# LeSN-Lab/diff-ViT

Measured on AMD Instinct MI355X. Metric: images/sec DeiT-S int8 224^2 b=256 (quantized forward), higher is better.
Workload: dtype int8; 1 GPU; deit_small PoT-PTQ forward, bit_config=[8]*50, 224x224, batch 256 per GPU; global_batch=256, parallelism=dp1, streams_per_gpu=3, collective=none, ranks_seen=1, distinct_devices=1

## Files before the change

diff-vit_amd/csrc/p2vit_attn.hip:

```cpp
#include "p2vit_attn_lis.h"

#define WA_HD 32
#define WA_KEYS 64
#define WA_DEAD(kb, r) (NT > 0 && (kb) * 16 + (r) >= NT)
#define WA_PAD(kb, r) (!(NT > 0 && (kb) * 16 + 12 + (r) < NT))
template <int NT, bool TAP>
__global__ __launch_bounds__(256, 3) void k_window_attention(WinAttnArgs a) {
  constexpr int VSTRIDE = WA_KEYS + 4;
  __shared__ __attribute__((aligned(16))) int8_t sK[4][WA_KEYS * WA_HD];
  __shared__ __attribute__((aligned(16))) unsigned short sVt[4][WA_HD * VSTRIDE];
  __shared__ float sT[4][232];
  __shared__ __attribute__((aligned(16))) unsigned short sP[4][4][16];
  __shared__ unsigned short sMeta[WA_KEYS + 16];
  __shared__ long long lutE[258];
  __shared__ double lutFR[258];
  const int tid = threadIdx.x, lane = tid & 63, wave = tid >> 6, g = lane >> 4, l15 = lane & 15;
  const int ws = a.wa.ws, N = ws * ws, nW = a.wa.n_windows;
  const int hgroups = (a.H + 3) >> 2;
  const int blk = blockIdx.x;
  const int hg = blk % hgroups, w = (blk / hgroups) % nW, b = blk / (hgroups * nW);
  const int head = hg * 4 + wave;
  const int C = a.H * WA_HD;
  const long long ldq = a.wa.qkv_stride ? a.wa.qkv_stride : 3 * C, ldo = a.wa.out_stride ? a.wa.out_stride : C;
  const bool hok = head < a.H;
// ... 244 lines not shown
  const int hgroups = (a.H + 3) / 4;
  const dim3 grid((unsigned)(a.B * a.wa.n_windows * hgroups));
  if (a.wa.ws == 7) {
    if (a.probs_k) hipLaunchKernelGGL((k_window_attention<49, true>), grid, dim3(256), 0, st, a);
    else hipLaunchKernelGGL((k_window_attention<49, false>), grid, dim3(256), 0, st, a);
  } else {
    if (a.probs_k) hipLaunchKernelGGL((k_window_attention<0, true>), grid, dim3(256), 0, st, a);
    else hipLaunchKernelGGL((k_window_attention<0, false>), grid, dim3(256), 0, st, a);
  }
  CHECK_LAUNCH();
  return 0;
}

int p2v_launch_attention_wide(const AttnArgs& a, int head_dim, int nkb, hipStream_t st);

int g_attn_stream = 0;
int p2v_launch_attention(const AttnArgs& a, int head_dim, hipStream_t st) {
  const int nkb = (a.N + 31) / 32;
  {
    int ex;
    const float m2 = a.at.s_qkv_sq * a.at.inv_s_attn;
    if (!(m2 > 0.f) || frexpf(m2, &ex) != 0.5f) return -2;
  }
  if (g_attn_stream || a.N > p2v_resident_tokens_of(head_dim)) return p2v_launch_attention_stream(a, head_dim, st);
  if (head_dim == 64) { P2V_ATTN_CASES(64, 19, true) }
  if (head_dim == 32) { P2V_ATTN_CASES(32, 19, false) }
  return p2v_launch_attention_wide(a, head_dim, nkb, st);
}
```

diff-vit_amd/csrc/p2vit_attn_lis.h:

```cpp
#pragma once
#include "p2vit_device.h"

extern int g_attn_waves;


#define P2V_PROB_SCALE 0x1p111f
__device__ __forceinline__ unsigned lis_prob_pair(float r0, float r1) {
  const unsigned hi2 = __builtin_amdgcn_perm(__float_as_uint(r1), __float_as_uint(r0), 0x07060302u);
  const unsigned eb = __builtin_bit_cast(unsigned, __builtin_bit_cast(v2u16, hi2) + (v2u16){0x40, 0x40}) & 0x7F807F80u;
  unsigned out;
  asm("v_pk_sub_u16 %0, %1, %2 clamp" : "=v"(out) : "s"(0x47804780u), "v"(eb));
  return out;
}

#ifdef P2V_DIAG
extern unsigned long long* g_gemm_stamps;
#define AT_STAMP(slot)                                                                                             \
  do {                                                                                                             \
    if (a.stamps && threadIdx.x == 0 && (slot) < 16) a.stamps[(long long)blockIdx.x * 16 + (slot)] = __builtin_readcyclecounter(); \
  } while (0)
#else
#define AT_STAMP(slot) do { } while (0)
#endif
template <int HD, int NKP, bool TAP, bool ISH>
__global__ __launch_bounds__(512, HD > 64 ? 2 : (NKP <= 7 ? 4 : (NKP <= 10 ? 3 : 2))) void k_lis_attention(AttnArgs a) {
  static_assert(HD % 16 == 0 && HD >= 16 && HD <= 128, "head_dim");
  constexpr int KROWS = NKP * 32;
  constexpr int NKB = NKP * 2;
  constexpr int VSTRIDE = KROWS + 4;
// ... 3 lines not shown
  extern __shared__ __attribute__((aligned(16))) unsigned char smem[];
  int8_t* sK = reinterpret_cast<int8_t*>(smem);
  unsigned short* sVt = reinterpret_cast<unsigned short*>(smem + KROWS * HD);
  unsigned char* lutE = smem + KROWS * HD + HD * VSTRIDE * 2;
  unsigned char* lutFR = lutE + 258 * 8;
  typedef __attribute__((address_space(3))) const long long* lds_i64p;
  typedef __attribute__((address_space(3))) const double* lds_f64p;
  const int ebase = (int)(unsigned)(uintptr_t)(__attribute__((address_space(3))) unsigned char*)lutE;

  const int tid = threadIdx.x, lane = tid & 63, wave = tid >> 6, g = lane >> 4, l15 = lane & 15;
  const int b = blockIdx.x / a.H, head = blockIdx.x % a.H;
  const int N = a.N, D = a.H * HD, ld = 3 * D;
  const int8_t* base = a.qkv + (long long)b * N * ld + head * HD;
  AT_STAMP(0);

  if (tid < 256) {
    int xi = -tid;
    const int lim = 32 * a.at.x0_int;
    xi = xi < lim ? lim : xi;
    const int q = xi / a.at.x0_int;
    const int r = xi - a.at.x0_int * q;
    const long long z = (long long)r * (r + a.at.b_int) + a.at.c_int;
    long long e = z << (32 - q);
    e = e < 0 ? 0 : e;
    const float ef = (float)e;
    reinterpret_cast<long long*>(lutE)[tid] = e;
    reinterpret_cast<double*>(lutFR)[tid] = 1.0 / (double)ef;
    if (tid == 0) {
      reinterpret_cast<long long*>(lutE)[256] = 0;
      reinterpret_cast<double*>(lutFR)[256] = 1.0;
    }
  }
  AT_STAMP(1);
  for (int i0 = tid; i0 < KROWS * CH; i0 += 2 * (int)blockDim.x) {
    uint4 kv[2], vv[2];
#pragma unroll
    for (int u = 0; u < 2; ++u) {
      const int i = i0 + u * (int)blockDim.x;
      const int row = i / CH, c = i % CH;
      kv[u] = make_uint4(0, 0, 0, 0);
      vv[u] = make_uint4(0, 0, 0, 0);
      if (i < KROWS * CH && row < N) {
        kv[u] = *reinterpret_cast<const uint4*>(base + (long long)row * ld + D + c * 16);
        vv[u] = *reinterpret_cast<const uint4*>(base + (long long)row * ld + 2 * D + c * 16);
      }
    }
#pragma unroll
    for (int u = 0; u < 2; ++u) {
      const int i = i0 + u * (int)blockDim.x;
      if (i >= KROWS * CH) break;
      const int row = i / CH, c = i % CH;
      const int sw = (HD == 64) ? (c ^ (((row >> 3) & 1) << 1)) : c;
      *reinterpret_cast<uint4*>(sK + row * HD + sw * 16) = kv[u];
      const unsigned w4[4] = {vv[u].x, vv[u].y, vv[u].z, vv[u].w};
#pragma unroll
      for (int j = 0; j < 16; ++j) {
        const float f = (float)sx8(w4[j >> 2], j & 3);
        sVt[(c * 16 + j) * VSTRIDE + row] = (unsigned short)(__float_as_uint(f) >> 16);
      }
// ... 31 lines not shown
    v4i s[NKB];
#pragma unroll
    for (int kb = 0; kb < NKB; ++kb) {
      const int row = kb * 16 + l15;
#pragma unroll
      for (int j = 0; j < NQ; ++j) {
        const bool live = 4 * j + g < CH;
        const int c = live ? 4 * j + g : 0;
        const int sw = (HD == 64) ? (c ^ (((row >> 3) & 1) << 1)) : c;
        v4i fk = *reinterpret_cast<const v4i*>(sK + row * HD + sw * 16);
        if (!live) fk = (v4i){0, 0, 0, 0};
        if (j == 0) s[kb] = __builtin_amdgcn_mfma_i32_16x16x64_i8(fk, fq[0], (v4i){0, 0, 0, 0}, 0, 0, 0);
        else s[kb] = __builtin_amdgcn_mfma_i32_16x16x64_i8(fk, fq[j], s[kb], 0, 0, 0);
      }
    }
    const bool tail_empty = (NKB - 1) * 16 >= N;
#ifdef P2V_DIAG
    asm volatile("s_nop 0" :: "v"(s[NKB - 1][0]));
#endif
    AT_STAMP(stamp_base);
    long long S = 0;
    if (ISH) {
      const int p = a.pshift, hm1 = (1 << (p - 1)) - 1;
      int mx = -100000;
#pragma unroll
      for (int kb = 0; kb < NKB; ++kb) {
        if (kb == NKB - 1 && tail_empty) continue;
#pragma unroll
        for (int r = 0; r < 4; ++r) {
          const int sv = s[kb][r];
          int code = (int)((unsigned)sv + (unsigned)hm1 + (((unsigned)sv >> p) & 1u)) >> p;
          code = code < -128 ? -128 : (code > 127 ? 127 : code);
          if (kb >= NKB - 2) code = (kb * 16 + 4 * g + r) < N ? code : -100000;
          s[kb][r] = code;
          mx = code > mx ? code : mx;
        }
      }
      {
        int o = __shfl_xor(mx, 16);
        mx = o > mx ? o : mx;
        o = __shfl_xor(mx, 32);
        mx = o > mx ? o : mx;
      }
      const int mx8 = (mx << 3) + ebase;
#pragma unroll
      for (int kb = 0; kb < NKB; ++kb) {
        if (kb == NKB - 1 && tail_empty) continue;
#pragma unroll
        for (int r = 0; r < 4; ++r) {
          int d8;
          asm("v_mad_i32_i24 %0, %1, -8, %2" : "=v"(d8) : "v"(s[kb][r]), "v"(mx8));
          if (kb >= NKB - 2) d8 = d8 > ebase + 2048 ? ebase + 2048 : d8;
          s[kb][r] = d8;
          S += *(lds_i64p)(uintptr_t)(unsigned)d8;
        }
        __builtin_amdgcn_sched_barrier(0);
      }
    } else {
    int mn = 1000;
#pragma unroll
    for (int kb = 0; kb < NKB; ++kb) {
      if (kb == NKB - 1 && tail_empty) continue;
#pragma unroll
      for (int r = 0; r < 4; ++r) {
        int nc = (int)__builtin_amdgcn_fmed3f(rintf((float)s[kb][r] * nmm), -127.f, 128.f);
        if (kb >= NKB - 2) nc = (kb * 16 + 4 * g + r) < N ? nc : 1000;
        s[kb][r] = nc;
        mn = nc < mn ? nc : mn;
      }
    }
    {
      int o = __shfl_xor(mn, 16);
      mn = o < mn ? o : mn;
      o = __shfl_xor(mn, 32);
      mn = o < mn ? o : mn;
    }
    const int neg8mn = -8 * mn + ebase;
#pragma unroll
    for (int kb = 0; kb < NKB; ++kb) {
      if (kb == NKB - 1 && tail_empty) continue;
#pragma unroll
      for (int r = 0; r < 4; ++r) {
        int d8 = (s[kb][r] << 3) + neg8mn;
        if (kb >= NKB - 2) d8 = d8 > ebase + 2048 ? ebase + 2048 : d8;
        s[kb][r] = d8;
        S += *(lds_i64p)(uintptr_t)(unsigned)d8;
      }
      __builtin_amdgcn_sched_barrier(0);
    }
    }
    S += __shfl_xor(S, 16);
    S += __shfl_xor(S, 32);
    const float Sf = (float)S;
    const double Sd = (double)Sf;
    AT_STAMP(stamp_base + 1);

    v4f o[NDT];
#pragma unroll
    for (int dt = 0; dt < NDT; ++dt) o[dt] = (v4f){0.f, 0.f, 0.f, 0.f};
#pragma unroll
    for (int p = 0; p < NKP; ++p) {
      unsigned pk[4];
#pragma unroll
      for (int e2 = 0; e2 < 4; ++e2) {
        float ratio[2];
#pragma unroll
        for (int e = 0; e < 2; ++e) {
          const int j = 2 * e2 + e;
          const int kb = 2 * p + (j >> 2), r = j & 3;
          if (kb == NKB - 1 && tail_empty) {
            ratio[e] = 4.0e9f;
            continue;
          }
          const double rd = ((lds_f64p)(uintptr_t)(unsigned)s[kb][r])[258];
          ratio[e] = rintf((float)(Sd * rd));
          if (TAP && s[kb][r] < ebase + 2048 && qrow < N) {
            int k = (int)((__float_as_uint(ratio[e]) + 0x00400000u) >> 23) - 127;
            a.probs_k[(((long long)b * a.H + head) * N + qrow) * N + kb * 16 + 4 * g + r] = (int8_t)(k > 16 ? 16 : k);
          }
        }
        pk[e2] = lis_prob_pair(ratio[0], ratio[1]);
      }
      v4i pb = {(int)pk[0], (int)pk[1], (int)pk[2], (int)pk[3]};
      const v8bf fb = __builtin_bit_cast(v8bf, pb);
#pragma unroll
      for (int dt = 0; dt < NDT; ++dt) {
        const unsigned short* vp = sVt + (dt * 16 + l15) * VSTRIDE + p * 32 + 4 * g;
        const uint2 lo = *reinterpret_cast<const uint2*>(vp);
        const uint2 hi = *reinterpret_cast<const uint2*>(vp + 16);
        v4i va = {(int)lo.x, (int)lo.y, (int)hi.x, (int)hi.y};
        o[dt] = __builtin_amdgcn_mfma_f32_16x16x32_bf16(__builtin_bit_cast(v8bf, va), fb, o[dt], 0, 0, 0);
      }
      __builtin_amdgcn_sched_barrier(0);
    }
#ifdef P2V_DIAG
    asm volatile("s_nop 0" :: "v"(o[NDT - 1][0]));
#endif
    AT_STAMP(stamp_base + 2);
    {
      const int qs = qrow < N ? qrow : N - 1;
      int8_t* dst = a.out + ((long long)b * N + qs) * D + head * HD + 4 * g;
#pragma unroll
      for (int dt = 0; dt < NDT; ++dt)
        *reinterpret_cast<unsigned*>(dst + dt * 16) = pack4_rne_sat(o[dt][0] * avm, o[dt][1] * avm, o[dt][2] * avm, o[dt][3] * avm);
    }
    AT_STAMP(stamp_base + 3);
    stamp_base += 4;
  }
}

template <int HD, int NKB, bool ISH_OK = true>
static int launch_attn_t(const AttnArgs& a_, hipStream_t st) {
  constexpr int KROWS = NKB * 32;
  constexpr size_t smem = (size_t)KROWS * HD + (size_t)HD * (KROWS + 4) * 2 + 258 * 8 + 258 * 8;
  AttnArgs a = a_;
  {
    int ex;
    const float m = a.at.qk_scale * (a.at.s_qkv_sq * a.at.inv_s_attn);
    a.pshift = (m > 0.f && frexpf(m, &ex) == 0.5f && ex <= 0 && ex >= -23) ? 1 - ex : 0;
  }
#ifdef P2V_DIAG
  a.stamps = g_gemm_stamps;
#endif
// ... 40 lines not shown
```

diff-vit_amd/csrc/p2vit_capi.cpp:

```cpp
#include <hip/hip_runtime.h>
#include <math.h>
#include <stdarg.h>
#include <stdio.h>
#include <stdlib.h>
#include <string.h>

#include <vector>

#include "p2vit_kernels.h"

static thread_local char g_err[512] = "";

static int fail(int code, const char* fmt, ...) {
  va_list ap;
  va_start(ap, fmt);
  vsnprintf(g_err, sizeof g_err, fmt, ap);
  va_end(ap);
  return code;
}
static int launch_rc(int rc, const char* what) {
  if (rc == 0) return 0;
  if (rc == -2) return fail(P2V_E_UNSUPPORTED, "%s: s_qkv_sq * inv_s_attn must be a power of two", what);
  if (rc < 0) return fail(P2V_E_UNSUPPORTED, "%s: no kernel instantiated for this shape", what);
  return fail(P2V_E_LAUNCH, "%s: %s", what, hipGetErrorString((hipError_t)rc));
// ... 37 lines not shown
  std::vector<char> lin_set[2];
  float inv_s_input;
  p2v_epilogue embed_epi;
  const int8_t* cls_codes;
  bool embed_set;
  std::vector<p2v_block> blocks;
  std::vector<char> block_set;
  p2v_ln final_ln;
  float head_inv_s, head_s;
  bool head_set;
  std::vector<float*> ln_pre_buf;
  float* final_pre_buf = nullptr;
  std::vector<char> block_folded;
  std::vector<const float*> resid_tab;
  std::vector<float*> resid_buf;
  int device = -1;
  ~p2v_plan() {
    int prev = -1;
    const bool sw = device >= 0 && hipGetDevice(&prev) == hipSuccess && prev != device && hipSetDevice(device) == hipSuccess;
    for (float* b : ln_pre_buf)
      if (b) (void)hipFree(b);
    for (float* b : resid_buf)
      if (b) (void)hipFree(b);
    if (final_pre_buf) (void)hipFree(final_pre_buf);
    if (sw) (void)hipSetDevice(prev);
  }
};

static void build_resid_tables(p2v_plan* plan, int block);
static int bit_index(int bits) { return bits == 4 ? 0 : (bits == 8 ? 1 : -1); }

extern "C" {

extern int g_ln_generic;
extern int g_ln_rows;
extern int g_attn_waves;
extern int g_ln_gemm;
extern int g_ln_gemm_ver;
extern int g_gemm_tile;
extern int g_resid_pre;
extern int g_attn_stream;
extern int g_ln_pre;
extern int g_gemm_rows;
int g_cls_rows = 1;
// ... 70 lines not shown
  p->patches = (d.img_size / d.patch_size) * (d.img_size / d.patch_size);
  p->tokens = p->patches + 1;
  p->k_patch = d.in_chans * d.patch_size * d.patch_size;
  p->k_patch_pad = round_up(p->k_patch, GBK_PAD);
  p->n_layers = 4 * d.depth + 2;
  for (int b = 0; b < 2; ++b) {
    p->lin[b].assign(p->n_layers, p2v_linear{nullptr, nullptr, nullptr, nullptr, 0});
    p->lin_set[b].assign(p->n_layers, 0);
  }
  p->blocks.resize(d.depth);
  p->block_set.assign(d.depth, 0);
  p->ln_pre_buf.assign(d.depth, nullptr);
  p->block_folded.assign(d.depth, 0);
  p->resid_tab.assign((size_t)d.depth * 4, nullptr);
  p->resid_buf.assign(d.depth, nullptr);
  p->embed_set = p->head_set = false;
  p->cls_codes = nullptr;
  *out = p;
  return P2V_OK;
}

void p2v_plan_destroy(p2v_plan* plan) { delete plan; }

int p2v_plan_set_linear(p2v_plan* plan, int layer, int bits, const p2v_linear* lin) {
  if (!plan || !lin) return fail(P2V_E_ARG, "p2v_plan_set_linear: null argument");
  const int bi = bit_index(bits);
  if (bi < 0) return fail(P2V_E_BITS, "bits %d not in {4, 8}", bits);
  if (layer < 0 || layer >= plan->n_layers) return fail(P2V_E_ARG, "layer %d out of range [0,%d)", layer, plan->n_layers);
  if (!lin->w_codes || !lin->colscale || !lin->bias) return fail(P2V_E_ARG, "p2v_plan_set_linear: null device pointer");
  if (lin->packed4 && bits != 4) return fail(P2V_E_BITS, "packed4 weights for a %d-bit layer", bits);
// ... 70 lines not shown
  const size_t per = resid_tab_floats(D);
  if (hipDeviceSynchronize() != hipSuccess) { (void)hipGetLastError(); return; }
  float* buf = plan->resid_buf[block];
  if (!buf && hipMalloc(&buf, 4 * per * sizeof(float)) != hipSuccess) { (void)hipGetLastError(); return; }
  plan->resid_buf[block] = buf;
  plan->device = dev.own;
  for (int which = 0; which < 2; ++which)
    for (int bi = 0; bi < 2; ++bi) {
      const int layer = 1 + 4 * block + (which ? 3 : 1);
      if (!plan->lin_set[bi][layer]) continue;
      int usable = 0;
      float* tab = buf + (size_t)(which * 2 + bi) * per;
      if (resid_prefold_impl(plan->lin[bi][layer], which ? blk.fc2_epi : blk.proj_epi, D, tab, &usable, nullptr) == P2V_OK && usable)
        plan->resid_tab[(size_t)block * 4 + which * 2 + bi] = tab;
    }
}

static hipError_t fold_one_ln(const p2v_ln& l, int C, float* dev, p2v_ln_pre* out) {
  const int Cp = round_up(C, 256);
  std::vector<float> g(C), b(C), io(C), pm(C), host((size_t)2 * Cp, 0.f);
  hipError_t e = hipMemcpy(g.data(), l.gamma, C * sizeof(float), hipMemcpyDeviceToHost);
  if (e == hipSuccess) e = hipMemcpy(b.data(), l.beta, C * sizeof(float), hipMemcpyDeviceToHost);
  if (e == hipSuccess) e = hipMemcpy(io.data(), l.inv_out, C * sizeof(float), hipMemcpyDeviceToHost);
  if (e == hipSuccess) e = hipMemcpy(pm.data(), l.post_mul, C * sizeof(float), hipMemcpyDeviceToHost);
  if (e != hipSuccess) return e;
  float* go = host.data();
  float* bo = go + Cp;
  int pot = 1, pm1 = 1;
  float gmin = 3.0e38f, gmax = 0.f, bmax = 0.f;
  for (int c = 0; c < C; ++c) {
// ... 61 lines not shown
                       !blk->fc2_epi.s_next))
    rc = fail(P2V_E_ARG, "p2v_plan_set_block: RESID epilogues need s_mid/s_res/s_next");
  for (int i = 0; i < 6 && rc == P2V_OK; ++i) {
    const p2v_ln& l = i < 2 ? blk->ln1[i] : blk->ln2[(i - 2) >> 1][(i - 2) & 1];
    if (!l.mask || !l.gamma || !l.beta || !l.inv_out || !l.post_mul) rc = fail(P2V_E_ARG, "p2v_plan_set_block: LayerNorm constants missing");
  }
  if (rc != P2V_OK) return rc;
  plan->blocks[block] = *blk;
  plan->block_set[block] = 1;
  g_err[0] = 0;
  plan->block_folded[block] = fold_ln_constants(plan, block) ? 1 : 0;
  {
    char keep[sizeof g_err];
    memcpy(keep, g_err, sizeof keep);
    build_resid_tables(plan, block);
    memcpy(g_err, keep, sizeof keep);
  }
  return P2V_OK;
}

int p2v_plan_block_prefolded(const p2v_plan* plan, int block) {
  if (!plan || block < 0 || block >= plan->d.depth) return fail(P2V_E_ARG, "p2v_plan_block_prefolded: bad argument");
  return plan->block_folded[block] ? 1 : 0;
}

int p2v_plan_resid_prefolded(const p2v_plan* plan, int block) {
  if (!plan || block < 0 || block >= plan->d.depth) return fail(P2V_E_ARG, "p2v_plan_resid_prefolded: bad argument");
  int m = 0;
  for (int j = 0; j < 4; ++j) m |= plan->resid_tab[(size_t)block * 4 + j] ? 1 << j : 0;
  return m;
}

int p2v_plan_set_head(p2v_plan* plan, const p2v_ln* final_ln, float inv_s_out, float s_out) {
// ... 228 lines not shown
    LnArgs ln{bufX, D, M, D, b.ln1[bq], bufLN, D};
    ln.pre = b.ln1[bq].pre;
    p2v_epilogue e{};
    e.inv_s_out = b.inv_s_qkv[bq];
    e.tap_out = qkv_tap ? qkv_tap[i] : (lin_tap ? lin_tap[1 + 4 * i] : nullptr);
    if (p->lin[bq][1 + 4 * i].w_frag && p2v_ln_gemm_supported(P2V_EPI_REQUANT, D, 3 * D, 0)) {
      if (!taps) ln.out = nullptr;
      STEP(P2V_K_LN_GEMM_QKV, run_ln_gemm(P2V_EPI_REQUANT, ln, p->lin[bq][1 + 4 * i], e, 3 * D, bufQKV, st));
    } else {
      STEP(P2V_K_LAYERNORM, launch_rc(p2v_launch_layernorm(ln, st), "int_layernorm"));
      STEP(P2V_K_GEMM_QKV, run_gemm(P2V_EPI_REQUANT, bufLN, D, M, Dk, 3 * D, p->lin[bq][1 + 4 * i], e, bufQKV, 3 * D, nullptr, st));
    }
    DDV_TAP(T, 3 * D);
    DDV_I8(bufQKV, T, 3 * D, nullptr);
    AttnArgs at{bufQKV, batch, T, d.num_heads, b.attn, bufATT, nullptr};
    p2v_epilogue ep = b.proj_epi;
    ep.residual = bufX;
    ep.resid_tab = p->resid_tab[(size_t)i * 4 + bp];
    if (i == d.depth - 1 && cls_only) {
      const long long TD = (long long)T * D;
      at.nq = 1;
      STEP(P2V_K_ATTENTION, launch_rc(p2v_launch_attention(at, hd, st), "lis_attention"));
      STEP(P2V_K_GEMM_PROJ, run_gemm_few_rows(P2V_EPI_RESID, bufATT, (int)TD, batch, Dk, D, p->lin[bp][2 + 4 * i], ep, bufX, (int)TD, st));
      LnArgs lc{bufX, TD, batch, D, b.ln2[bq][b1], bufLN, D};
      lc.pre = b.ln2[bq][b1].pre;
      STEP(P2V_K_LAYERNORM, launch_rc(p2v_launch_layernorm(lc, st), "int_layernorm"));
      p2v_epilogue e1{};
      e1.inv_s_out = b.inv_s_fc1;
      e1.gelu = b.gelu_fc1;
      STEP(P2V_K_GEMM_FC1, run_gemm_few_rows(P2V_EPI_GELU, bufLN, D, batch, Dk, Hd, p->lin[b1][3 + 4 * i], e1, bufHID, Hd, st));
// ... 252 lines not shown

int p2v_lis_attention_rows(const int8_t* qkv, int batch, int tokens, int heads, int head_dim, const p2v_attn* at, int query_rows,
                           int8_t* out, void* stream) {
  if (!qkv || !at || !out) return fail(P2V_E_ARG, "p2v_lis_attention_rows: null argument");
  if (batch <= 0 || tokens <= 0 || heads <= 0) return fail(P2V_E_SHAPE, "bad attention shape");
  if (query_rows < 1 || query_rows > tokens) return fail(P2V_E_SHAPE, "p2v_lis_attention_rows: query_rows %d outside 1 .. %d", query_rows, tokens);
  {
    const int rc = check_attn("p2v_lis_attention_rows", *at);
    if (rc != P2V_OK) return rc;
  }
  AttnArgs a{qkv, batch, tokens, heads, *at, out, nullptr};
  a.nq = query_rows;
  return launch_rc(p2v_launch_attention(a, head_dim, (hipStream_t)stream), "lis_attention");
}

int p2v_patch_merge_gather(const int8_t* x, int batch, int H, int W, int C, int8_t* out, void* stream) {
  if (!x || !out) return fail(P2V_E_ARG, "p2v_patch_merge_gather: null argument");
  if (batch <= 0 || H <= 0 || W <= 0 || (H & 1) || (W & 1)) return fail(P2V_E_SHAPE, "patch merge: H and W must be positive and even");
  if (C <= 0 || C % 16) return fail(P2V_E_UNSUPPORTED, "patch merge: C must be a multiple of 16");
  return launch_rc(p2v_launch_patch_merge_gather(x, batch, H, W, C, out, (hipStream_t)stream), "patch_merge_gather");
}

int p2v_avgpool_quant(const int8_t* x, int batch, int tokens, int C, float s_in, float inv_s_out, int8_t* out, void* stream) {
  if (!x || !out) return fail(P2V_E_ARG, "p2v_avgpool_quant: null argument");
  if (batch <= 0 || tokens <= 0 || tokens > 8192) return fail(P2V_E_SHAPE, "avgpool: bad shape");
  if (C <= 0 || C % 4) return fail(P2V_E_UNSUPPORTED, "avgpool: C must be a multiple of 4");
  return launch_rc(p2v_launch_avgpool_quant(x, batch, tokens, C, s_in, inv_s_out, out, (hipStream_t)stream), "avgpool_quant");
}

int p2v_window_attention(const int8_t* qkv, int batch, int tokens_per_image, int heads, int head_dim, const p2v_winattn* wa,
// ... 269 lines not shown
```

diff-vit_amd/csrc/p2vit_kernels.h:

```cpp
#pragma once
#include <hip/hip_runtime.h>
#include <stdint.h>

#include "../../include/p2vit.h"

#define GBK_PAD 64
#define P2V_EPI_F32 7

struct GemmArgs {
  const int8_t* A;
  int lda, M;
  const int8_t* W;
  int K, N;
  int w4;
  const float* colscale;
  const float* bias;
  p2v_epilogue ep;
  void* out;
  int ldo;
  int8_t* out_codes;
  int tiles_n;
#ifdef P2V_DIAG
  unsigned long long* stamps;
#endif
// ... 10 lines not shown
  int8_t* out;
  long long out_stride;
  int rows_per_half;
  int force_generic;
  LnPre pre;
};

struct AttnArgs {
  const int8_t* qkv;
  int B, N, H;
  p2v_attn at;
  int8_t* out;
  int8_t* probs_k;
  int pshift;
  int nq;
#ifdef P2V_DIAG
  unsigned long long* stamps;
#endif
};

struct WinAttnArgs {
  const int8_t* qkv;
  int B, T, H;
  p2v_winattn wa;
  int8_t* out;
  int8_t* probs_k;
};
int p2v_launch_patch_merge_gather(const int8_t* x, int B, int H, int W, int C, int8_t* out, hipStream_t st);
int p2v_launch_avgpool_quant(const int8_t* x, int B, int T, int C, float s_in, float inv_s_out, int8_t* out, hipStream_t st);
int p2v_launch_window_attention(const WinAttnArgs& a, hipStream_t st);

int p2v_launch_patchify(const float* img, int B, int C, int H, int W, int P, float inv_s, int8_t* out, int k_pad, hipStream_t st);
int p2v_launch_fill_cls(int8_t* x, int B, int T, int D, const int8_t* cls, hipStream_t st);
int p2v_launch_embed_fp32(const float* img, int B, int C, int H, int W, int P, const GemmArgs& g, hipStream_t st);
int p2v_launch_u8_patchify(const uint8_t* img, int B, int C, int H, int W, int P, int nhwc, const int8_t* lut, int8_t* out, int k_pad,
                           hipStream_t st);
int p2v_launch_embed_u8(const uint8_t* img, int nhwc, const float* lut, int B, int C, int H, int W, int P, const GemmArgs& g, hipStream_t st);
int p2v_launch_gemm(int epi, const GemmArgs& g, hipStream_t st);
int p2v_launch_gemm_rows(int epi, const GemmArgs& g, hipStream_t st);
int p2v_launch_resid_prefold(const p2v_linear& lin, const p2v_epilogue& ep, int N, float* tab, unsigned* flags, hipStream_t st);
int p2v_launch_layernorm(const LnArgs& a, hipStream_t st);
bool p2v_ln_gemm_supported(int epi, int C, int N, int table_cells);
int p2v_launch_ln_gemm(int epi, const LnArgs& a, const GemmArgs& g, hipStream_t st);
int p2v_launch_attention(const AttnArgs& a, int head_dim, hipStream_t st);
int p2v_launch_attention_stream(const AttnArgs& a, int head_dim, hipStream_t st);
inline int p2v_resident_tokens_of(int head_dim) {
  if (head_dim == 32 || head_dim == 48 || head_dim == 64 || head_dim == 80) return P2V_MAX_TOKENS;
  return head_dim == 96 ? 17 * 32 : (head_dim == 128 ? 12 * 32 : 0);
}
int p2v_launch_stream_probe(int kernels, int usec, int workgroups, int lds_bytes, hipStream_t st);
int p2v_launch_fake_quant(const float* x, long long n, const float* scale, int n_scale, long long inner, int lo, int hi,
                          float* out, int8_t* codes, hipStream_t st);
int p2v_launch_gelu_quant(const float* y, long long n, float inv_s, int8_t* codes, unsigned long long* flags, int force_slow,
                          hipStream_t st);
int p2v_launch_gelu_sweep(unsigned first_bits, unsigned count, float* max_err, hipStream_t st);
int p2v_launch_gelu_table_build(float inv_s, const p2v_gelu_tab& t, unsigned* scratch, hipStream_t st);
int p2v_launch_gelu_table_check(float inv_s, const p2v_gelu_tab& t, unsigned long long* mismatches, hipStream_t st);

#include <vector>
// ... 37 lines not shown
```

diff-vit_amd/engine.py:

```python
import ctypes as C
import os

_HERE = os.path.dirname(os.path.abspath(__file__))
LIB_PATH = os.path.join(_HERE, 'csrc', 'libp2vit_hip.so')

P2V_ABI_VERSION = 6
EPI_REQUANT, EPI_GELU, EPI_RESID, EPI_EMBED, EPI_HEAD = 0, 1, 2, 3, 4
E_ARG, E_BITS, E_SHAPE, E_UNSUPPORTED, E_WORKSPACE, E_LAUNCH, E_STATE = -1, -2, -3, -4, -5, -6, -7
LAYOUT_NCHW, LAYOUT_NHWC = 0, 1
LAYOUTS = {'NCHW': LAYOUT_NCHW, 'NHWC': LAYOUT_NHWC}

KERNEL_KINDS = ('patchify', 'gemm_embed', 'fill_cls', 'layernorm', 'gemm_qkv', 'attention', 'gemm_proj', 'gemm_fc1',
                'gemm_fc2', 'gemm_head', 'ln_gemm_qkv', 'ln_gemm_fc1', 'event_gap')

_f, _i, _p, _ll = C.c_float, C.c_int32, C.c_void_p, C.c_longlong


class ModelDesc(C.Structure):
    _fields_ = [('abi_version', _i), ('img_size', _i), ('patch_size', _i), ('in_chans', _i), ('embed_dim', _i),
                ('depth', _i), ('num_heads', _i), ('mlp_hidden', _i), ('num_classes', _i)]


class Linear(C.Structure):
    _fields_ = [('w_codes', _p), ('colscale', _p), ('bias', _p), ('w_frag', _p), ('packed4', _i)]
# ... 111 lines not shown
        L.p2v_ddv_tap_scratch_bytes.argtypes = [_p, _i]
        L.p2v_ddv_tap_scratch_bytes.restype = C.c_size_t
        L.p2v_forward_ddv.argtypes = [_p, _p, _i, C.POINTER(C.c_int8), _i, _p, _p, C.c_size_t, _i, _p, C.c_size_t, _p, _p]
    L.p2v_forward_profile.argtypes = [_p, _p, _i, C.POINTER(C.c_int8), _i, _p, _p, C.c_size_t, _p, C.POINTER(C.c_float),
                                      C.POINTER(C.c_int32), _i]
    L.p2v_forward_profile_begin.argtypes = [_p, _p, _i, C.POINTER(C.c_int8), _i, _p, _p, C.c_size_t, _p, C.POINTER(_p)]
    L.p2v_forward_profile_end.argtypes = [_p, C.POINTER(C.c_float), C.POINTER(C.c_int32), _i]
    L.p2v_quantize_patchify.argtypes = [_p, _i, _i, _i, _i, _i, _f, _p, _i, _p]
    L.p2v_forward_u8.argtypes = [_p, _p, _i, _p, _i, C.POINTER(C.c_int8), _i, _p, _p, C.c_size_t, _i, _p]
    L.p2v_u8_patchify.argtypes = [_p, _i, _p, _i, _i, _i, _i, _i, _p, _i, _p]
    L.p2v_gemm_i8.argtypes = [_i, _p, _i, _i, _i, _i, C.POINTER(Linear), C.POINTER(Epilogue), _p, _i, _p, _p]
    L.p2v_int_layernorm.argtypes = [_p, _ll, _i, _i, C.POINTER(Ln), _p, _ll, _p]
    L.p2v_lis_attention.argtypes = [_p, _i, _i, _i, _i, C.POINTER(Attn), _p, _p, _p]
    if hasattr(L, 'p2v_lis_attention_rows'):
        L.p2v_lis_attention_rows.argtypes = [_p, _i, _i, _i, _i, C.POINTER(Attn), _i, _p, _p]
    L.p2v_ln_gemm_i8.argtypes = [_i, _p, _ll, _i, _i, C.POINTER(Ln), _i, C.POINTER(Linear), C.POINTER(Epilogue), _p, _i, _p, _p]
    L.p2v_ln_gemm_fusable.argtypes = [_i, _i, _i, _i]
    L.p2v_set_tuning.argtypes = [C.c_char_p, _i]
    L.p2v_ln_gemm_fusable.restype = _i
    L.p2v_run_ops.argtypes = [C.POINTER(Op), _i, _p]
    L.p2v_run_ops_profile.argtypes = [C.POINTER(Op), _i, _p, C.POINTER(C.c_float)]
    L.p2v_patch_merge_gather.argtypes = [_p, _i, _i, _i, _i, _p, _p]
    L.p2v_avgpool_quant.argtypes = [_p, _i, _i, _i, _f, _f, _p, _p]
    L.p2v_window_attention.argtypes = [_p, _i, _i, _i, _i, C.POINTER(WinAttn), _p, _p, _p]
    L.p2v_fake_quant_f32.argtypes = [_p, _ll, _p, _i, _ll, _i, _i, _p, _p, _p]
    L.p2v_gelu_quant_f32.argtypes = [_p, _ll, _f, _p, _p, _i, _p]
    L.p2v_gelu_err_sweep.argtypes = [C.c_uint32, C.c_uint32, _p, _p]
    L.p2v_stream_probe.argtypes = [_p, C.c_int, C.c_int, C.c_int, C.c_int]
    L.p2v_gelu_table_plan.argtypes = [_f, C.POINTER(GeluTab)]
    L.p2v_gelu_table_scratch_bytes.argtypes = [_i]
# ... 197 lines not shown
```

include/p2vit.h:

```cpp
#ifndef P2VIT_H
#define P2VIT_H

#include <stddef.h>
#include <stdint.h>

#ifdef __cplusplus
extern "C" {
#endif

#define P2V_ABI_VERSION 6
#define P2V_MAX_TOKENS 608
#define P2V_MAX_TOKENS_STREAMED 4096
int p2v_max_tokens(int head_dim);
int p2v_resident_tokens(int head_dim);

enum {
  P2V_OK = 0,
  P2V_E_ARG = -1,
  P2V_E_BITS = -2,
  P2V_E_SHAPE = -3,
  P2V_E_UNSUPPORTED = -4,
  P2V_E_WORKSPACE = -5,
  P2V_E_LAUNCH = -6,
  P2V_E_STATE = -7
// ... 86 lines not shown
                       const int8_t* cls_row_codes );

typedef struct p2v_block {
  p2v_ln ln1[2];
  float inv_s_qkv[2];
  p2v_attn attn;
  p2v_epilogue proj_epi;
  p2v_ln ln2[2][2];
  float inv_s_fc1;
  p2v_gelu_tab gelu_fc1;
  p2v_epilogue fc2_epi;
} p2v_block;
int p2v_plan_set_block(p2v_plan* plan, int block, const p2v_block* blk);
int p2v_plan_block_prefolded(const p2v_plan* plan, int block);
int p2v_plan_resid_prefolded(const p2v_plan* plan, int block);

int p2v_plan_set_head(p2v_plan* plan, const p2v_ln* final_ln, float inv_s_out, float s_out);

size_t p2v_workspace_bytes(const p2v_plan* plan, int batch);

int p2v_forward(p2v_plan* plan, const float* images, int batch, const int8_t* bit_config, int n_cfg,
                float* logits, void* workspace, size_t workspace_bytes, int stop_after, void* stream);

int p2v_forward_taps(p2v_plan* plan, const float* images, int batch, const int8_t* bit_config, int n_cfg,
                     float* logits, void* workspace, size_t workspace_bytes, float* const* qkv_out, float* const* fc1_out,
                     void* stream);

int p2v_forward_linear_taps(p2v_plan* plan, const float* images, int batch, const int8_t* bit_config, int n_cfg,
                            float* logits, void* ws, size_t ws_bytes, float* const* taps, void* stream);

// ... 28 lines not shown

int p2v_gemm_i8(int epilogue_kind, const int8_t* A, int lda, int M, int K, int N, const p2v_linear* lin,
                const p2v_epilogue* epi, void* out, int ldo, int8_t* out_codes, void* stream);

int p2v_int_layernorm(const int8_t* x, long long row_stride, int rows, int C, const p2v_ln* ln,
                      int8_t* out, long long out_stride, void* stream);

int p2v_ln_gemm_i8(int epilogue_kind, const int8_t* x, long long row_stride, int M, int C, const p2v_ln* ln, int N,
                   const p2v_linear* lin, const p2v_epilogue* epi, int8_t* out, int ldo, int8_t* ln_out, void* stream);
int p2v_ln_gemm_fusable(int epilogue_kind, int C, int N, int gelu_table_cells);

int p2v_lis_attention(const int8_t* qkv, int batch, int tokens, int heads, int head_dim, const p2v_attn* at,
                      int8_t* out, int8_t* probs_k, void* stream);
int p2v_lis_attention_rows(const int8_t* qkv, int batch, int tokens, int heads, int head_dim, const p2v_attn* at, int query_rows,
                           int8_t* out, void* stream);

typedef struct p2v_winattn {
  float s_q1;
  float qk_scale;
  float s_attn;
  float s_table;
  float s_q2;
  float s_q3;
  int32_t x0_int, b_int, c_int;
  const int8_t* table_codes;
  const int32_t* win_index;
  const int8_t* region;
  int32_t ws, n_windows;
  int32_t qkv_stride;
  int32_t out_stride;
// ... 83 lines not shown
```

Measured before the change: 111,200 images/sec.

## Precompute LIS softmax tables per block and trim tail-key work in attention

Each attention block used to compute its exp and reciprocal lookup tables in LDS on every launch, which includes an integer divide and a double-precision reciprocal. The plan now builds them once per layer in device memory, and the kernel just copies them in. The kernel also permutes the keys in the partial last 16-key tile, so live keys sit in the low register slots. The tail loops then run only over live slots, and requantisation uses a float-magic-number path. This adds plan-time device buffers and more complex index handling for the tail keys and the probs tap writes, which risks subtle ordering bugs.

```diff
diff --git a/diff-vit_amd/csrc/p2vit_attn.hip b/diff-vit_amd/csrc/p2vit_attn.hip
--- a/diff-vit_amd/csrc/p2vit_attn.hip
+++ b/diff-vit_amd/csrc/p2vit_attn.hip
@@ -282,6 +282,21 @@
 
 int p2v_launch_attention_wide(const AttnArgs& a, int head_dim, int nkb, hipStream_t st);
 
+static __global__ void k_lis_tables(int x0_int, int b_int, int c_int, unsigned long long* tab) {
+  const int d = threadIdx.x;
+  if (d >= P2V_LIS_TAB_ENTRIES) return;
+  long long e = 0;
+  double fr = 0.0;
+  if (d <= 256) lis_table_entry(d, x0_int, b_int, c_int, &e, &fr);
+  tab[d] = (unsigned long long)e;
+  tab[P2V_LIS_TAB_ENTRIES + d] = __builtin_bit_cast(unsigned long long, fr);
+}
+int p2v_launch_attn_tables(const p2v_attn& at, unsigned long long* tab, hipStream_t st) {
+  hipLaunchKernelGGL(k_lis_tables, dim3(1), dim3(320), 0, st, at.x0_int, at.b_int, at.c_int, tab);
+  CHECK_LAUNCH();
+  return 0;
+}
+
 int g_attn_stream = 0;
 int p2v_launch_attention(const AttnArgs& a, int head_dim, hipStream_t st) {
   const int nkb = (a.N + 31) / 32;
diff --git a/diff-vit_amd/csrc/p2vit_attn_lis.h b/diff-vit_amd/csrc/p2vit_attn_lis.h
--- a/diff-vit_amd/csrc/p2vit_attn_lis.h
+++ b/diff-vit_amd/csrc/p2vit_attn_lis.h
@@ -13,6 +13,37 @@
   return out;
 }
 
+#define P2V_REQ_MAGIC 0x4B400000
+#define P2V_REQ_PAD 0x4B000000
+__device__ __forceinline__ int lis_requant_bits(int sv, float two_mp) {
+  const int bits = __float_as_int(__builtin_fmaf((float)sv, two_mp, 12582912.f));
+  const int lo = P2V_REQ_MAGIC - 128, hi = P2V_REQ_MAGIC + 127;
+  return bits < lo ? lo : (bits > hi ? hi : bits);
+}
+
+#define P2V_LIS_TAB_ENTRIES 258
+static_assert(P2V_ATTN_TAB_BYTES == 2 * P2V_LIS_TAB_ENTRIES * 8, "table layout");
+__device__ __forceinline__ void lis_table_entry(int d, int x0_int, int b_int, int c_int, long long* e_out, double* fr_out) {
+  if (d >= 256) {
+    *e_out = 0;
+    *fr_out = 1.0;
+    return;
+  }
+  int xi = -d;
+  const int lim = 32 * x0_int;
+  xi = xi < lim ? lim : xi;
+  const int q = xi / x0_int;
+  const int r = xi - x0_int * q;
+  const long long z = (long long)r * (r + b_int) + c_int;
+  long long e = z << (32 - q);
+  e = e < 0 ? 0 : e;
+  const float ef = (float)e;
+  *e_out = e;
+  *fr_out = 1.0 / (double)ef;
+}
+__device__ __forceinline__ int lis_key_of(int row, int N) {
+  return (row >> 4) == (N >> 4) ? (row & ~15) + 4 * (row & 3) + ((row >> 2) & 3) : row;
+}
 #ifdef P2V_DIAG
 extern unsigned long long* g_gemm_stamps;
 #define AT_STAMP(slot)                                                                                             \
@@ -46,21 +77,12 @@
   const int8_t* base = a.qkv + (long long)b * N * ld + head * HD;
   AT_STAMP(0);
 
-  if (tid < 256) {
-    int xi = -tid;
-    const int lim = 32 * a.at.x0_int;
-    xi = xi < lim ? lim : xi;
-    const int q = xi / a.at.x0_int;
-    const int r = xi - a.at.x0_int * q;
-    const long long z = (long long)r * (r + a.at.b_int) + a.at.c_int;
-    long long e = z << (32 - q);
-    e = e < 0 ? 0 : e;
-    const float ef = (float)e;
-    reinterpret_cast<long long*>(lutE)[tid] = e;
-    reinterpret_cast<double*>(lutFR)[tid] = 1.0 / (double)ef;
-    if (tid == 0) {
-      reinterpret_cast<long long*>(lutE)[256] = 0;
-      reinterpret_cast<double*>(lutFR)[256] = 1.0;
+  for (int d = tid; d <= 256; d += (int)blockDim.x) {
+    if (a.tab) {
+      reinterpret_cast<unsigned long long*>(lutE)[d] = a.tab[d];
+      reinterpret_cast<unsigned long long*>(lutFR)[d] = a.tab[P2V_LIS_TAB_ENTRIES + d];
+    } else {
+      lis_table_entry(d, a.at.x0_int, a.at.b_int, a.at.c_int, reinterpret_cast<long long*>(lutE) + d, reinterpret_cast<double*>(lutFR) + d);
     }
   }
   AT_STAMP(1);
@@ -69,12 +91,12 @@
 #pragma unroll
     for (int u = 0; u < 2; ++u) {
       const int i = i0 + u * (int)blockDim.x;
-      const int row = i / CH, c = i % CH;
+      const int c = i % CH, key = lis_key_of(i / CH, N);
       kv[u] = make_uint4(0, 0, 0, 0);
       vv[u] = make_uint4(0, 0, 0, 0);
-      if (i < KROWS * CH && row < N) {
-        kv[u] = *reinterpret_cast<const uint4*>(base + (long long)row * ld + D + c * 16);
-        vv[u] = *reinterpret_cast<const uint4*>(base + (long long)row * ld + 2 * D + c * 16);
+      if (i < KROWS * CH && key < N) {
+        kv[u] = *reinterpret_cast<const uint4*>(base + (long long)key * ld + D + c * 16);
+        vv[u] = *reinterpret_cast<const uint4*>(base + (long long)key * ld + 2 * D + c * 16);
       }
     }
 #pragma unroll
@@ -136,27 +158,34 @@
         else s[kb] = __builtin_amdgcn_mfma_i32_16x16x64_i8(fk, fq[j], s[kb], 0, 0, 0);
       }
     }
-    const bool tail_empty = (NKB - 1) * 16 >= N;
+    const int tlive = (N - 16 * (NKB - 2) + 3) >> 2;
+#define LIS_LANE_KEY(kb, r) ((kb) * 16 + 4 * (r) + g < N)
 #ifdef P2V_DIAG
     asm volatile("s_nop 0" :: "v"(s[NKB - 1][0]));
 #endif
     AT_STAMP(stamp_base);
     long long S = 0;
     if (ISH) {
-      const int p = a.pshift, hm1 = (1 << (p - 1)) - 1;
-      int mx = -100000;
-#pragma unroll
-      for (int kb = 0; kb < NKB; ++kb) {
-        if (kb == NKB - 1 && tail_empty) continue;
+      const float two_mp = __uint_as_float((unsigned)(127 - a.pshift) << 23);
+      int mx = P2V_REQ_PAD;
+#pragma unroll
+      for (int kb = 0; kb < NKB - 2; ++kb) {
 #pragma unroll
         for (int r = 0; r < 4; ++r) {
-          const int sv = s[kb][r];
-          int code = (int)((unsigned)sv + (unsigned)hm1 + (((unsigned)sv >> p) & 1u)) >> p;
-          code = code < -128 ? -128 : (code > 127 ? 127 : code);
-          if (kb >= NKB - 2) code = (kb * 16 + 4 * g + r) < N ? code : -100000;
+          const int code = lis_requant_bits(s[kb][r], two_mp);
           s[kb][r] = code;
           mx = code > mx ? code : mx;
         }
+        if (NKP > 10) __builtin_amdgcn_sched_barrier(0);
+      }
+#pragma unroll
+      for (int ts = 0; ts < 8; ++ts) {
+        if (ts >= tlive) break;
+        const int kb = NKB - 2 + (ts >> 2), r = ts & 3;
+        int code = lis_requant_bits(s[kb][r], two_mp);
+        code = LIS_LANE_KEY(kb, r) ? code : P2V_REQ_PAD;
+        s[kb][r] = code;
+        mx = code > mx ? code : mx;
       }
       {
         int o = __shfl_xor(mx, 16);
@@ -164,52 +193,77 @@
         o = __shfl_xor(mx, 32);
         mx = o > mx ? o : mx;
       }
-      const int mx8 = (mx << 3) + ebase;
-#pragma unroll
-      for (int kb = 0; kb < NKB; ++kb) {
-        if (kb == NKB - 1 && tail_empty) continue;
+      const int mx8 = (int)(((unsigned)mx << 3) - 0x58000000u + (unsigned)ebase);
+#pragma unroll
+      for (int kb = 0; kb < NKB - 2; ++kb) {
 #pragma unroll
         for (int r = 0; r < 4; ++r) {
           int d8;
           asm("v_mad_i32_i24 %0, %1, -8, %2" : "=v"(d8) : "v"(s[kb][r]), "v"(mx8));
-          if (kb >= NKB - 2) d8 = d8 > ebase + 2048 ? ebase + 2048 : d8;
           s[kb][r] = d8;
           S += *(lds_i64p)(uintptr_t)(unsigned)d8;
         }
         __builtin_amdgcn_sched_barrier(0);
       }
+#pragma unroll
+      for (int ts = 0; ts < 8; ++ts) {
+        if (ts >= tlive) break;
+        const int kb = NKB - 2 + (ts >> 2), r = ts & 3;
+        int d8;
+        asm("v_mad_i32_i24 %0, %1, -8, %2" : "=v"(d8) : "v"(s[kb][r]), "v"(mx8));
+        d8 = d8 > ebase + 2048 ? ebase + 2048 : d8;
+        s[kb][r] = d8;
+        S += *(lds_i64p)(uintptr_t)(unsigned)d8;
+      }
+      __builtin_amdgcn_sched_barrier(0);
     } else {
-    int mn = 1000;
-#pragma unroll
-    for (int kb = 0; kb < NKB; ++kb) {
-      if (kb == NKB - 1 && tail_empty) continue;
-#pragma unroll
-      for (int r = 0; r < 4; ++r) {
+      int mn = 1000;
+#pragma unroll
+      for (int kb = 0; kb < NKB - 2; ++kb) {
+#pragma unroll
+        for (int r = 0; r < 4; ++r) {
+          const int nc = (int)__builtin_amdgcn_fmed3f(rintf((float)s[kb][r] * nmm), -127.f, 128.f);
+          s[kb][r] = nc;
+          mn = nc < mn ? nc : mn;
+        }
+        if (NKP > 10) __builtin_amdgcn_sched_barrier(0);
+      }
+#pragma unroll
+      for (int ts = 0; ts < 8; ++ts) {
+        if (ts >= tlive) break;
+        const int kb = NKB - 2 + (ts >> 2), r = ts & 3;
         int nc = (int)__builtin_amdgcn_fmed3f(rintf((float)s[kb][r] * nmm), -127.f, 128.f);
-        if (kb >= NKB - 2) nc = (kb * 16 + 4 * g + r) < N ? nc : 1000;
+        nc = LIS_LANE_KEY(kb, r) ? nc : 1000;
         s[kb][r] = nc;
         mn = nc < mn ? nc : mn;
       }
-    }
-    {
-      int o = __shfl_xor(mn, 16);
-      mn = o < mn ? o : mn;
-      o = __shfl_xor(mn, 32);
-      mn = o < mn ? o : mn;
-    }
-    const int neg8mn = -8 * mn + ebase;
-#pragma unroll
-    for (int kb = 0; kb < NKB; ++kb) {
-      if (kb == NKB - 1 && tail_empty) continue;
-#pragma unroll
-      for (int r = 0; r < 4; ++r) {
+      {
+        int o = __shfl_xor(mn, 16);
+        mn = o < mn ? o : mn;
+        o = __shfl_xor(mn, 32);
+        mn = o < mn ? o : mn;
+      }
+      const int neg8mn = -8 * mn + ebase;
+#pragma unroll
+      for (int kb = 0; kb < NKB - 2; ++kb) {
+#pragma unroll
+        for (int r = 0; r < 4; ++r) {
+          const int d8 = (s[kb][r] << 3) + neg8mn;
+          s[kb][r] = d8;
+          S += *(lds_i64p)(uintptr_t)(unsigned)d8;
+        }
+        __builtin_amdgcn_sched_barrier(0);
+      }
+#pragma unroll
+      for (int ts = 0; ts < 8; ++ts) {
+        if (ts >= tlive) break;
+        const int kb = NKB - 2 + (ts >> 2), r = ts & 3;
         int d8 = (s[kb][r] << 3) + neg8mn;
-        if (kb >= NKB - 2) d8 = d8 > ebase + 2048 ? ebase + 2048 : d8;
+        d8 = d8 > ebase + 2048 ? ebase + 2048 : d8;
         s[kb][r] = d8;
         S += *(lds_i64p)(uintptr_t)(unsigned)d8;
       }
       __builtin_amdgcn_sched_barrier(0);
-    }
     }
     S += __shfl_xor(S, 16);
     S += __shfl_xor(S, 32);
@@ -222,23 +276,24 @@
     for (int dt = 0; dt < NDT; ++dt) o[dt] = (v4f){0.f, 0.f, 0.f, 0.f};
 #pragma unroll
     for (int p = 0; p < NKP; ++p) {
-      unsigned pk[4];
+      unsigned pk[4] = {0u, 0u, 0u, 0u};
 #pragma unroll
       for (int e2 = 0; e2 < 4; ++e2) {
+        if (p == NKP - 1 && 2 * e2 >= tlive) break;
         float ratio[2];
 #pragma unroll
         for (int e = 0; e < 2; ++e) {
           const int j = 2 * e2 + e;
           const int kb = 2 * p + (j >> 2), r = j & 3;
-          if (kb == NKB - 1 && tail_empty) {
-            ratio[e] = 4.0e9f;
-            continue;
-          }
+          ratio[e] = 4.0e9f;
+          if (p == NKP - 1 && j >= tlive) continue;
           const double rd = ((lds_f64p)(uintptr_t)(unsigned)s[kb][r])[258];
           ratio[e] = rintf((float)(Sd * rd));
           if (TAP && s[kb][r] < ebase + 2048 && qrow < N) {
             int k = (int)((__float_as_uint(ratio[e]) + 0x00400000u) >> 23) - 127;
-            a.probs_k[(((long long)b * a.H + head) * N + qrow) * N + kb * 16 + 4 * g + r] = (int8_t)(k > 16 ? 16 : k);
+            int8_t* pk_row = a.probs_k + (((long long)b * a.H + head) * N + qrow) * N;
+            if (kb >= NKB - 2 && kb == (N >> 4)) pk_row[g + (kb * 16 + 4 * r)] = (int8_t)(k > 16 ? 16 : k);
+            else pk_row[4 * g + (kb * 16 + r)] = (int8_t)(k > 16 ? 16 : k);
           }
         }
         pk[e2] = lis_prob_pair(ratio[0], ratio[1]);
@@ -269,6 +324,7 @@
     AT_STAMP(stamp_base + 3);
     stamp_base += 4;
   }
+#undef LIS_LANE_KEY
 }
 
 template <int HD, int NKB, bool ISH_OK = true>
diff --git a/diff-vit_amd/csrc/p2vit_capi.cpp b/diff-vit_amd/csrc/p2vit_capi.cpp
--- a/diff-vit_amd/csrc/p2vit_capi.cpp
+++ b/diff-vit_amd/csrc/p2vit_capi.cpp
@@ -75,6 +75,7 @@
   std::vector<char> block_folded;
   std::vector<const float*> resid_tab;
   std::vector<float*> resid_buf;
+  std::vector<unsigned long long*> attn_tab;
   int device = -1;
   ~p2v_plan() {
     int prev = -1;
@@ -83,12 +84,15 @@
       if (b) (void)hipFree(b);
     for (float* b : resid_buf)
       if (b) (void)hipFree(b);
+    for (unsigned long long* b : attn_tab)
+      if (b) (void)hipFree(b);
     if (final_pre_buf) (void)hipFree(final_pre_buf);
     if (sw) (void)hipSetDevice(prev);
   }
 };
 
 static void build_resid_tables(p2v_plan* plan, int block);
+static void build_attn_tables(p2v_plan* plan, int block);
 static int bit_index(int bits) { return bits == 4 ? 0 : (bits == 8 ? 1 : -1); }
 
 extern "C" {
@@ -189,6 +193,7 @@
   p->block_folded.assign(d.depth, 0);
   p->resid_tab.assign((size_t)d.depth * 4, nullptr);
   p->resid_buf.assign(d.depth, nullptr);
+  p->attn_tab.assign(d.depth, nullptr);
   p->embed_set = p->head_set = false;
   p->cls_codes = nullptr;
   *out = p;
@@ -289,6 +294,22 @@
       if (resid_prefold_impl(plan->lin[bi][layer], which ? blk.fc2_epi : blk.proj_epi, D, tab, &usable, nullptr) == P2V_OK && usable)
         plan->resid_tab[(size_t)block * 4 + which * 2 + bi] = tab;
     }
+}
+
+static void build_attn_tables(p2v_plan* plan, int block) {
+  unsigned long long* buf = plan->attn_tab[block];
+  plan->attn_tab[block] = nullptr;
+  OwnerDevice dev(plan->blocks[block].ln1[0].gamma);
+  bool ok = dev.ok() && (plan->device < 0 || plan->device == dev.own);
+  if (ok && !buf && hipMalloc(&buf, P2V_ATTN_TAB_BYTES) != hipSuccess) { buf = nullptr; ok = false; }
+  if (ok) ok = p2v_launch_attn_tables(plan->blocks[block].attn, buf, nullptr) == 0 && hipStreamSynchronize(nullptr) == hipSuccess;
+  if (ok) {
+    plan->device = dev.own;
+    plan->attn_tab[block] = buf;
+    return;
+  }
+  (void)hipGetLastError();
+  if (buf && dev.ok()) (void)hipFree(buf);
 }
 
 static hipError_t fold_one_ln(const p2v_ln& l, int C, float* dev, p2v_ln_pre* out) {
@@ -380,9 +401,15 @@
     char keep[sizeof g_err];
     memcpy(keep, g_err, sizeof keep);
     build_resid_tables(plan, block);
+    build_attn_tables(plan, block);
     memcpy(g_err, keep, sizeof keep);
   }
   return P2V_OK;
+}
+
+int p2v_plan_attn_tables(const p2v_plan* plan, int block) {
+  if (!plan || block < 0 || block >= plan->d.depth) return fail(P2V_E_ARG, "p2v_plan_attn_tables: bad argument");
+  return plan->attn_tab[block] ? 1 : 0;
 }
 
 int p2v_plan_block_prefolded(const p2v_plan* plan, int block) {
@@ -641,6 +668,7 @@
     DDV_TAP(T, 3 * D);
     DDV_I8(bufQKV, T, 3 * D, nullptr);
     AttnArgs at{bufQKV, batch, T, d.num_heads, b.attn, bufATT, nullptr};
+    at.tab = p->attn_tab[i];
     p2v_epilogue ep = b.proj_epi;
     ep.residual = bufX;
     ep.resid_tab = p->resid_tab[(size_t)i * 4 + bp];
@@ -923,6 +951,42 @@
   return launch_rc(p2v_launch_attention(a, head_dim, (hipStream_t)stream), "lis_attention");
 }
 
+size_t p2v_attn_tables_bytes(void) { return P2V_ATTN_TAB_BYTES; }
+
+int p2v_attn_tables(const p2v_attn* at, void* tab, size_t tab_bytes, void* stream) {
+  if (!at || !tab) return fail(P2V_E_ARG, "p2v_attn_tables: null argument");
+  if (tab_bytes < P2V_ATTN_TAB_BYTES) return fail(P2V_E_WORKSPACE, "p2v_attn_tables: table needs %d bytes, got %zu", (int)P2V_ATTN_TAB_BYTES, tab_bytes);
+  if ((uintptr_t)tab & 7) return fail(P2V_E_ARG, "p2v_attn_tables: the table must be 8-byte aligned");
+  {
+    const int rc = check_attn("p2v_attn_tables", *at);
+    if (rc != P2V_OK) return rc;
+  }
+  {
+    hipPointerAttribute_t pa;
+    if (hipPointerGetAttributes(&pa, tab) != hipSuccess || (pa.type != hipMemoryTypeDevice && pa.type != hipMemoryTypeManaged)) {
+      (void)hipGetLastError();
+      return fail(P2V_E_ARG, "p2v_attn_tables: tab is not device memory");
+    }
+  }
+  return launch_rc(p2v_launch_attn_tables(*at, (unsigned long long*)tab, (hipStream_t)stream), "attn_tables");
+}
+
+int p2v_lis_attention_tab(const int8_t* qkv, int batch, int tokens, int heads, int head_dim, const p2v_attn* at, const void* tab,
+                          int query_rows, int8_t* out, int8_t* probs_k, void* stream) {
+  if (!qkv || !at || !out) return fail(P2V_E_ARG, "p2v_lis_attention_tab: null argument");
+  if (batch <= 0 || tokens <= 0 || heads <= 0) return fail(P2V_E_SHAPE, "bad attention shape");
+  if (query_rows < 0 || query_rows > tokens) return fail(P2V_E_SHAPE, "p2v_lis_attention_tab: query_rows %d outside 0 .. %d", query_rows, tokens);
+  if ((uintptr_t)tab & 7) return fail(P2V_E_ARG, "p2v_lis_attention_tab: the table must be 8-byte aligned");
+  {
+    const int rc = check_attn("p2v_lis_attention_tab", *at);
+    if (rc != P2V_OK) return rc;
+  }
+  AttnArgs a{qkv, batch, tokens, heads, *at, out, probs_k};
+  a.nq = query_rows;
+  a.tab = (const unsigned long long*)tab;
+  return launch_rc(p2v_launch_attention(a, head_dim, (hipStream_t)stream), "lis_attention");
+}
+
 int p2v_patch_merge_gather(const int8_t* x, int batch, int H, int W, int C, int8_t* out, void* stream) {
   if (!x || !out) return fail(P2V_E_ARG, "p2v_patch_merge_gather: null argument");
   if (batch <= 0 || H <= 0 || W <= 0 || (H & 1) || (W & 1)) return fail(P2V_E_SHAPE, "patch merge: H and W must be positive and even");
diff --git a/diff-vit_amd/csrc/p2vit_kernels.h b/diff-vit_amd/csrc/p2vit_kernels.h
--- a/diff-vit_amd/csrc/p2vit_kernels.h
+++ b/diff-vit_amd/csrc/p2vit_kernels.h
@@ -48,6 +48,7 @@
   int8_t* probs_k;
   int pshift;
   int nq;
+  const unsigned long long* tab;
 #ifdef P2V_DIAG
   unsigned long long* stamps;
 #endif
@@ -77,6 +78,8 @@
 bool p2v_ln_gemm_supported(int epi, int C, int N, int table_cells);
 int p2v_launch_ln_gemm(int epi, const LnArgs& a, const GemmArgs& g, hipStream_t st);
 int p2v_launch_attention(const AttnArgs& a, int head_dim, hipStream_t st);
+#define P2V_ATTN_TAB_BYTES (2 * 258 * 8)
+int p2v_launch_attn_tables(const p2v_attn& at, unsigned long long* tab, hipStream_t st);
 int p2v_launch_attention_stream(const AttnArgs& a, int head_dim, hipStream_t st);
 inline int p2v_resident_tokens_of(int head_dim) {
   if (head_dim == 32 || head_dim == 48 || head_dim == 64 || head_dim == 80) return P2V_MAX_TOKENS;
diff --git a/diff-vit_amd/engine.py b/diff-vit_amd/engine.py
--- a/diff-vit_amd/engine.py
+++ b/diff-vit_amd/engine.py
@@ -149,6 +149,12 @@
     L.p2v_lis_attention.argtypes = [_p, _i, _i, _i, _i, C.POINTER(Attn), _p, _p, _p]
     if hasattr(L, 'p2v_lis_attention_rows'):
         L.p2v_lis_attention_rows.argtypes = [_p, _i, _i, _i, _i, C.POINTER(Attn), _i, _p, _p]
+    if hasattr(L, 'p2v_lis_attention_tab'):
+        L.p2v_plan_attn_tables.argtypes = [_p, _i]
+        L.p2v_attn_tables_bytes.argtypes = []
+        L.p2v_attn_tables_bytes.restype = C.c_size_t
+        L.p2v_attn_tables.argtypes = [C.POINTER(Attn), _p, C.c_size_t, _p]
+        L.p2v_lis_attention_tab.argtypes = [_p, _i, _i, _i, _i, C.POINTER(Attn), _p, _i, _p, _p, _p]
     L.p2v_ln_gemm_i8.argtypes = [_i, _p, _ll, _i, _i, C.POINTER(Ln), _i, C.POINTER(Linear), C.POINTER(Epilogue), _p, _i, _p, _p]
     L.p2v_ln_gemm_fusable.argtypes = [_i, _i, _i, _i]
     L.p2v_set_tuning.argtypes = [C.c_char_p, _i]
diff --git a/include/p2vit.h b/include/p2vit.h
--- a/include/p2vit.h
+++ b/include/p2vit.h
@@ -124,6 +124,7 @@
 int p2v_plan_set_block(p2v_plan* plan, int block, const p2v_block* blk);
 int p2v_plan_block_prefolded(const p2v_plan* plan, int block);
 int p2v_plan_resid_prefolded(const p2v_plan* plan, int block);
+int p2v_plan_attn_tables(const p2v_plan* plan, int block);
 
 int p2v_plan_set_head(p2v_plan* plan, const p2v_ln* final_ln, float inv_s_out, float s_out);
 
@@ -182,6 +183,10 @@
                       int8_t* out, int8_t* probs_k, void* stream);
 int p2v_lis_attention_rows(const int8_t* qkv, int batch, int tokens, int heads, int head_dim, const p2v_attn* at, int query_rows,
                            int8_t* out, void* stream);
+size_t p2v_attn_tables_bytes(void);
+int p2v_attn_tables(const p2v_attn* at, void* tab, size_t tab_bytes, void* stream);
+int p2v_lis_attention_tab(const int8_t* qkv, int batch, int tokens, int heads, int head_dim, const p2v_attn* at, const void* tab,
+                          int query_rows, int8_t* out, int8_t* probs_k, void* stream);
 
 typedef struct p2v_winattn {
   float s_q1;
```

New measurement: 111,900 images/sec, median of 6. No clear change (+0.7%).
